# sohmandal/classpose

Measured on AMD Instinct MI355X. Metric: wsi_tiles_per_sec, higher is better.
Workload: dtype bf16; 1 GPU; configs[1]: synthetic 10000x10000 WSI (1936 tiles), tile 256 / overlap 32, conic 7 classes, ViT-L ClassTransformer depth 24 random-init, batch 32 sub-tiles = 8 WSI tiles/step, every step a distinct batch of the rank's shard (tiles sharded k % n_gpus, at most 256 distinct batches resident, longer runs wrap) streamed pinned host -> hipMemcpyAsync inside the timed region (the reader decodes ahead int; slide=10000, tile=256, overlap=32, batch_subtiles=32, distinct_batches=142, records_gathered=2048, decode_ahead_batches_at_t0=4, device_resident_batches_at_t0=1

## Files before the change

classpose_amd/csrc/cpx_gemm.hip:

```cpp
#include "cpx_internal.h"
#include <type_traits>

typedef __attribute__((ext_vector_type(8))) __bf16 bf16x8;
typedef __attribute__((ext_vector_type(8))) _Float16 f16x8;
typedef __attribute__((ext_vector_type(4))) float f32x4;

#define BM 128
#define BN 128
#define BK 64
#define GEMM_THREADS 256
#define TILE_BYTES (128 * 128)
#define STAGE_BYTES (2 * TILE_BYTES)

template <bool NT_POSSIBLE, bool WT_POSSIBLE = false>
__device__ __forceinline__ void st16(void *p, uint4 v, bool nt, bool wt = false) {
    if (WT_POSSIBLE && wt) {
        typedef unsigned u32x4_t __attribute__((ext_vector_type(4)));
        u32x4_t w = {v.x, v.y, v.z, v.w};
        if (NT_POSSIBLE && nt) asm volatile("global_store_dwordx4 %0, %1, off sc1 nt" ::"v"(p), "v"(w) : "memory");
        else asm volatile("global_store_dwordx4 %0, %1, off sc1" ::"v"(p), "v"(w) : "memory");
    } else if (NT_POSSIBLE && nt) {
        typedef unsigned u32x4_t __attribute__((ext_vector_type(4)));
        u32x4_t w = {v.x, v.y, v.z, v.w};
        __builtin_nontemporal_store(w, reinterpret_cast<u32x4_t *>(p));
// ... 228 lines not shown
                const size_t s_ = (size_t)(m >> 10), t_ = (size_t)(m & 1023);
#pragma unroll
                for (int r = 0; r < 4; ++r) {
                    const int c = n - 2048 + r;
                    vT[((s_ * 16 + (c >> 6)) * 64 + (c & 63)) * 1024 + t_] = to_half<F16>(v[r]);
                }
            } else {
                uint2 o;
                o.x = pack2<F16>(v[0], v[1]);
                o.y = pack2<F16>(v[2], v[3]);
                *reinterpret_cast<uint2 *>((unsigned short *)g.out + (size_t)m * g.ld_out + n) = o;
            }
        }
    }
}


typedef __attribute__((ext_vector_type(4))) unsigned u32x4;
#define G2_THREADS 512
#define G2_HALF 16384
#define G2_BUF 65536
#define G2_EPI_LD 528
#define G2_LN_OFF (256 * G2_EPI_LD)
#define G2_LDS_BYTES (G2_LN_OFF + 256 * 8)

template <int OFF>
__device__ __forceinline__ u32x4 lds_read128(unsigned addr) {
    u32x4 v;
    asm volatile("ds_read_b128 %0, %1 offset:%2" : "=v"(v) : "v"(addr), "n"(OFF));
    return v;
}
template <bool F16>
__device__ __forceinline__ f32x4 mfma16v(const u32x4 &a, const u32x4 &b, f32x4 c) {
    if constexpr (F16)
        return __builtin_amdgcn_mfma_f32_16x16x32_f16(__builtin_bit_cast(f16x8, a), __builtin_bit_cast(f16x8, b), c, 0, 0, 0);
    else
        return __builtin_amdgcn_mfma_f32_16x16x32_bf16(__builtin_bit_cast(bf16x8, a), __builtin_bit_cast(bf16x8, b), c, 0, 0, 0);
}
template <int HM>
__device__ __forceinline__ void g2_read_x(u32x4 (&fx)[4][2], unsigned b0, unsigned b1) {
    fx[0][0] = lds_read128<HM * G2_HALF + 0 * 2048>(b0); fx[0][1] = lds_read128<HM * G2_HALF + 0 * 2048>(b1);
    fx[1][0] = lds_read128<HM * G2_HALF + 1 * 2048>(b0); fx[1][1] = lds_read128<HM * G2_HALF + 1 * 2048>(b1);
    fx[2][0] = lds_read128<HM * G2_HALF + 2 * 2048>(b0); fx[2][1] = lds_read128<HM * G2_HALF + 2 * 2048>(b1);
    fx[3][0] = lds_read128<HM * G2_HALF + 3 * 2048>(b0); fx[3][1] = lds_read128<HM * G2_HALF + 3 * 2048>(b1);
}
template <int HN>
__device__ __forceinline__ void g2_read_w(u32x4 (&fw)[2][2], unsigned b0, unsigned b1) {
// ... 31 lines not shown
    int bid = blockIdx.x;
    {
        const int nxcd = 8, q = g.n_blocks / nxcd, r = g.n_blocks % nxcd, x = bid % nxcd;
        bid = (x < r ? x * (q + 1) : r * (q + 1) + (x - r) * q) + bid / nxcd;
    }
    int tile_m, tile_n;
    {
        const int tiles_m = g.n_blocks / g.tiles_n;
        if (g.l2_block && (tiles_m & 7) == 0 && (g.tiles_n & 3) == 0) {
            const int grp = bid >> 5, w_ = bid & 31, cgn = g.tiles_n >> 2, rgn = tiles_m >> 3;
            const int rg = g.l2_block == 2 ? grp % rgn : grp / cgn, cg = g.l2_block == 2 ? grp / rgn : grp - rg * cgn;
            tile_m = rg * 8 + (w_ >> 2);
            tile_n = cg * 4 + (w_ & 3);
        } else {
            tile_m = bid / g.tiles_n;
            tile_n = bid - tile_m * g.tiles_n;
        }
    }
    if (g.rev_m) tile_m = g.n_blocks / g.tiles_n - 1 - tile_m;
    const int m0 = tile_m * 256, n0 = tile_n * 256;
    const int K = g.K, nk = K / 64;

    const int srow = tid >> 3, kc = (tid & 7) ^ (srow & 7);
    const unsigned short *pX = g.A + (size_t)(m0 + srow) * K + kc * 8;
    const unsigned short *pW = g.W + (size_t)(n0 + srow) * K + kc * 8;
    const size_t k64 = (size_t)64 * K, k128 = (size_t)128 * K;
    char *sdst = smem + wave * 1024;
    auto stage = [&](int which, int t) {
        const unsigned short *p = (which < 2 ? pX : pW) + (which & 1) * k128 + (size_t)t * 64;
        char *d = sdst + (t & 1) * G2_BUF + which * G2_HALF;
        __builtin_amdgcn_global_load_lds((const __attribute__((address_space(1))) void *)p,
                                         (__attribute__((address_space(3))) void *)d, 16, 0, 0);
        __builtin_amdgcn_global_load_lds((const __attribute__((address_space(1))) void *)(p + k64),
                                         (__attribute__((address_space(3))) void *)(d + 8192), 16, 0, 0);
    };

    const unsigned lds0 = (unsigned)(size_t)(__attribute__((address_space(3))) char *)smem;
    unsigned xb[2][2], wb[2][2];
#pragma unroll
    for (int ks = 0; ks < 2; ++ks) {
        const unsigned sw = (unsigned)(((ks * 4 + fq) ^ (fr & 7)) << 4);
        xb[0][ks] = lds0 + (wm * 64 + fr) * 128 + sw;
        wb[0][ks] = lds0 + (wn * 32 + fr) * 128 + sw;
        xb[1][ks] = xb[0][ks] + G2_BUF;
        wb[1][ks] = wb[0][ks] + G2_BUF;
    }

    f32x4 acc[2][2][4][2];
#pragma unroll
    for (int a = 0; a < 2; ++a)
#pragma unroll
        for (int b = 0; b < 2; ++b)
#pragma unroll
            for (int c = 0; c < 4; ++c)
#pragma unroll
                for (int d = 0; d < 2; ++d) acc[a][b][c][d] = (f32x4){0.f, 0.f, 0.f, 0.f};
    u32x4 fx[4][2], fw[2][2];

    const bool ln_in = LN_IN && tid < 256;
    float4 st_a = make_float4(0.f, 0.f, 0.f, 0.f), st_b = st_a;
    if (ln_in) {
        st_a = *reinterpret_cast<const float4 *>(g.ln_stats + (size_t)(m0 + tid) * 8);
        st_b = *reinterpret_cast<const float4 *>(g.ln_stats + (size_t)(m0 + tid) * 8 + 4);
    }
    stage(0, 0); stage(2, 0); stage(3, 0); stage(1, 0);
    if (nk > 1) { stage(0, 1); stage(3, 1); }
    if (ln_in) {
        const float inv_k = 1.0f / K;
        const float sum = (st_a.x + st_a.z) + (st_b.x + st_b.z), sq = (st_a.y + st_a.w) + (st_b.y + st_b.w);
        const float mean = sum * inv_k;
        const float rstd = rsqrtf(fmaxf(sq * inv_k - mean * mean, 0.f) + 1e-6f);
        *reinterpret_cast<float2 *>(smem + G2_LN_OFF + tid * 8) = make_float2(rstd, -mean * rstd);
        asm volatile("s_waitcnt lgkmcnt(0)" ::: "memory");
    }
    if (nk > 1) asm volatile("s_waitcnt vmcnt(4)" ::: "memory");
    else asm volatile("s_waitcnt vmcnt(0)" ::: "memory");
    G2_BAR();
    if (wm == 1) G2_BAR();

#define G2_TILE(T, B)                                                                       \
    {                                                                                       \
        const int t_ = (T);                                                                 \
                                                                                    \
        g2_read_w<0>(fw, wb[B][0], wb[B][1]);                                               \
        g2_read_x<0>(fx, xb[B][0], xb[B][1]);                                               \
        if (t_ + 1 < nk) stage(1, t_ + 1);                                                  \
        G2_BAR(); G2_LGKM0();                                                               \
        g2_mma<F16>(acc[0][0], fx, fw);                                                     \
        __builtin_amdgcn_sched_barrier(0); G2_BAR();                                        \
                                                                                    \
        g2_read_w<1>(fw, wb[B][0], wb[B][1]);                                               \
        if (t_ + 1 < nk) stage(2, t_ + 1);                                                  \
        G2_BAR(); G2_LGKM0();                                                               \
        g2_mma<F16>(acc[0][1], fx, fw);                                                     \
        __builtin_amdgcn_sched_barrier(0); G2_BAR();                                        \
// ... 1 lines not shown
        g2_read_x<1>(fx, xb[B][0], xb[B][1]);                                               \
        if (t_ + 2 < nk) stage(0, t_ + 2);                                                  \
        G2_BAR(); G2_LGKM0();                                                               \
        g2_mma<F16>(acc[1][1], fx, fw);                                                     \
        __builtin_amdgcn_sched_barrier(0); G2_BAR();                                        \
                                                                                    \
        g2_read_w<0>(fw, wb[B][0], wb[B][1]);                                               \
        if (t_ + 2 < nk) { stage(3, t_ + 2); asm volatile("s_waitcnt vmcnt(4)" ::: "memory"); } \
        else if (t_ + 1 < nk) asm volatile("s_waitcnt vmcnt(0)" ::: "memory");              \
        G2_BAR(); G2_LGKM0();                                                               \
        g2_mma<F16>(acc[1][0], fx, fw);                                                     \
        __builtin_amdgcn_sched_barrier(0); G2_BAR();                                        \
    }

    for (int t = 0; t + 1 < nk; t += 2) {
        G2_TILE(t, 0)
        G2_TILE(t + 1, 1)
    }
    if (nk & 1) G2_TILE(nk - 1, 0)
#undef G2_TILE
    if (wm == 0) G2_BAR();
    __builtin_amdgcn_sched_barrier(0);

    const bool vt_tile = (EPI == CPX_EPI_QKV_BF16) && n0 >= 2048;
    const int c16 = tid & 31;
    float ln_mean[2][4], ln_rstd[2][4];
    if constexpr (LN_IN) {
#pragma unroll
        for (int hm = 0; hm < 2; ++hm)
#pragma unroll
            for (int mb = 0; mb < 4; ++mb) {
                const float2 p = *reinterpret_cast<const float2 *>(smem + G2_LN_OFF + (hm * 128 + wm * 64 + mb * 16 + fr) * 8);
                ln_rstd[hm][mb] = p.x; ln_mean[hm][mb] = p.y;
            }
    }
    uint4 rres[16];
    if constexpr (EPI == CPX_EPI_RESID_BF16) {
#pragma unroll
        for (int it = 0; it < 16; ++it)
            rres[it] = *reinterpret_cast<const uint4 *>((const unsigned short *)g.aux +
                                                        (size_t)(m0 + it * 16 + (tid >> 5)) * g.ld_out + n0 + c16 * 8);
    }
    float4 colb[2][2], colc[2][2];
#pragma unroll
    for (int hn = 0; hn < 2; ++hn)
#pragma unroll
        for (int nb = 0; nb < 2; ++nb) {
            const int nl = hn * 128 + wn * 32 + nb * 16 + fq * 4;
            colb[hn][nb] = g.bias ? *reinterpret_cast<const float4 *>(g.bias + n0 + nl) : make_float4(0.f, 0.f, 0.f, 0.f);
            if constexpr (LN_IN) colc[hn][nb] = *reinterpret_cast<const float4 *>(g.ln_colsum + n0 + nl);
        }
    auto convert_and_stage = [&](auto vt_tag) {
        constexpr bool VT = decltype(vt_tag)::value;
#pragma unroll
    for (int hm = 0; hm < 2; ++hm)
#pragma unroll
        for (int hn = 0; hn < 2; ++hn)
#pragma unroll
            for (int mb = 0; mb < 4; ++mb)
#pragma unroll
                for (int nb = 0; nb < 2; ++nb) {
                    const int ml = hm * 128 + wm * 64 + mb * 16 + fr;
                    const int nl = hn * 128 + wn * 32 + nb * 16 + fq * 4;
                    f32x4 v = acc[hm][hn][mb][nb];
                    const float4 b = colb[hn][nb];
                    if constexpr (LN_IN) {
                        const float4 cs = colc[hn][nb];
                        const float nm = ln_mean[hm][mb], rs = ln_rstd[hm][mb];
                        v[0] = fmaf(v[0], rs, fmaf(nm, cs.x, b.x)); v[1] = fmaf(v[1], rs, fmaf(nm, cs.y, b.y));
                        v[2] = fmaf(v[2], rs, fmaf(nm, cs.z, b.z)); v[3] = fmaf(v[3], rs, fmaf(nm, cs.w, b.w));
                    } else {
                        v[0] += b.x; v[1] += b.y; v[2] += b.z; v[3] += b.w;
                    }
                    if constexpr (EPI == CPX_EPI_GELU_BF16) {
#pragma unroll
                        for (int r = 0; r < 4; ++r) v[r] = gelu_erf(v[r]);
                    } else if constexpr (EPI == CPX_EPI_RELU_BF16) {
#pragma unroll
                        for (int r = 0; r < 4; ++r) v[r] = fmaxf(v[r], 0.f);
                    } else if constexpr (EPI == CPX_EPI_POS_BF16) {
                        const float4 pe = *reinterpret_cast<const float4 *>((const float *)g.aux + (size_t)((m0 + ml) & 1023) * g.N + n0 + nl);
                        v[0] += pe.x; v[1] += pe.y; v[2] += pe.z; v[3] += pe.w;
                    }
                    if constexpr (VT) {
                        const unsigned p01 = pack2<F16>(v[0], v[1]), p23 = pack2<F16>(v[2], v[3]);
                        *reinterpret_cast<unsigned short *>(smem + (nl + 0) * G2_EPI_LD + ml * 2) = (unsigned short)p01;
                        *reinterpret_cast<unsigned short *>(smem + (nl + 1) * G2_EPI_LD + ml * 2) = (unsigned short)(p01 >> 16);
                        *reinterpret_cast<unsigned short *>(smem + (nl + 2) * G2_EPI_LD + ml * 2) = (unsigned short)p23;
                        *reinterpret_cast<unsigned short *>(smem + (nl + 3) * G2_EPI_LD + ml * 2) = (unsigned short)(p23 >> 16);
                    } else {
                        uint2 o;
                        o.x = pack2<F16>(v[0], v[1]);
                        o.y = pack2<F16>(v[2], v[3]);
                        *reinterpret_cast<uint2 *>(smem + ml * G2_EPI_LD + nl * 2) = o;
                    }
                }
    };
    if (EPI == CPX_EPI_QKV_BF16 && vt_tile) convert_and_stage(std::true_type{});
    else convert_and_stage(std::false_type{});
    __syncthreads();
    if (vt_tile) {
        unsigned short *vT = (unsigned short *)g.aux;
        const size_t s_ = (size_t)(m0 >> 10), t0 = (size_t)(m0 & 1023);
#pragma unroll 4
        for (int it = 0; it < 16; ++it) {
            const int row = it * 16 + (tid >> 5);
            const int c = n0 - 2048 + row;
            uint4 v = *reinterpret_cast<const uint4 *>(smem + row * G2_EPI_LD + c16 * 16);
            *reinterpret_cast<uint4 *>(vT + ((s_ * 16 + (c >> 6)) * 64 + (c & 63)) * 1024 + t0 + c16 * 8) = v;
        }
    } else {
#pragma unroll
        for (int it = 0; it < 16; ++it) {
            const int ml = it * 16 + (tid >> 5);
            uint4 v = *reinterpret_cast<const uint4 *>(smem + ml * G2_EPI_LD + c16 * 16);
            const size_t go = (size_t)(m0 + ml) * g.ld_out + n0 + c16 * 8;
            if constexpr (EPI == CPX_EPI_RESID_BF16) {
                const uint4 rr = rres[it];
// ... 19 lines not shown
                if (c16 == 16)
                    *reinterpret_cast<float2 *>(g.stats_out + ((size_t)(m0 + ml) * LN_SLOTS + tile_n) * 2) = make_float2(sm, sq);
            }
        }
    }
}


#define G2P_STG_OFF G2_BUF
#define G2P_TAIL G2_LN_OFF
#define G2P_LDS_BYTES (G2_LN_OFF + 4096)
template <int EPI, bool F16, int FLAGS>
__global__ void __launch_bounds__(G2_THREADS, 2) k_gemm256p(GemmArgs g) {
    constexpr bool LN_IN = (FLAGS & G2F_LN) != 0 && EPI != CPX_EPI_RESID_BF16;
    constexpr bool STATS = (FLAGS & G2F_STATS) != 0 && EPI == CPX_EPI_RESID_BF16;
    extern __shared__ __attribute__((aligned(16))) char smem[];
    const int wave = __builtin_amdgcn_readfirstlane((int)threadIdx.x >> 6);
    const int wm = wave >> 2, wn = wave & 3;
    const int K = g.K, nk = K / 64, nblk = g.n_blocks, tiles_m = g.n_blocks / g.tiles_n;
    auto coords = [&](int v, int &m0_, int &n0_, int &tn_) {
        const int nxcd = 8, q = nblk / nxcd, r = nblk % nxcd, x = v % nxcd;
        int bid = (x < r ? x * (q + 1) : r * (q + 1) + (x - r) * q) + v / nxcd;
        int tile_m, tile_n;
        if (EPI == CPX_EPI_QKV_BF16 && g.l2_block == 3) {
            const int x = v & 7, slot = (v >> 3) & 31, i = v >> 8, rx = tiles_m >> 3, full = rx >> 4;
            int rg, cg;
            if (i < 6 * full) {
                const int rnd = i / 6, j = i - rnd * 6;
                rg = 2 * rnd + (j < 4 ? j >> 1 : j - 4); cg = j < 4 ? j & 1 : 2;
            } else {
                const int j = i - 6 * full;
                rg = 2 * full; cg = j < 2 ? j : 2;
            }
            tile_m = x * rx + rg * 8 + (slot >> 2);
            tile_n = cg * 4 + (slot & 3);
        } else if (g.l2_block && (tiles_m & 7) == 0 && (g.tiles_n & 3) == 0) {
            const int grp = bid >> 5, w_ = bid & 31, cgn = g.tiles_n >> 2, rgn = tiles_m >> 3;
            const int rg = g.l2_block == 2 ? grp % rgn : grp / cgn, cg = g.l2_block == 2 ? grp / rgn : grp - rg * cgn;
            tile_m = rg * 8 + (w_ >> 2);
            tile_n = cg * 4 + (w_ & 3);
        } else {
            tile_m = bid / g.tiles_n;
            tile_n = bid - tile_m * g.tiles_n;
        }
        if (g.rev_m) tile_m = tiles_m - 1 - tile_m;
        m0_ = tile_m * 256; n0_ = tile_n * 256; tn_ = tile_n;
    };
    char *sdst = smem + wave * 1024;
    const __amdgpu_buffer_rsrc_t rsrcX = __builtin_amdgcn_make_buffer_rsrc((void *)g.A, 0, 0x7FFFFFFF, 0x00020000);
    const __amdgpu_buffer_rsrc_t rsrcW = __builtin_amdgcn_make_buffer_rsrc((void *)g.W, 0, 0x7FFFFFFF, 0x00020000);
    const unsigned k64b = (unsigned)K * 128u, k128b = (unsigned)K * 256u;
    auto stage_at = [&](unsigned voff, unsigned sX, unsigned sW, int which, int t) {
        const unsigned so = (which < 2 ? sX : sW) + (which & 1) * k128b + (unsigned)t * 128u;
        char *d = sdst + (t & 1) * G2_BUF + which * G2_HALF;
        if (which < 2) {
            __builtin_amdgcn_raw_ptr_buffer_load_lds(rsrcX, (__attribute__((address_space(3))) void *)d, 16, voff, so, 0, 0);
            __builtin_amdgcn_raw_ptr_buffer_load_lds(rsrcX, (__attribute__((address_space(3))) void *)(d + 8192), 16, voff, so + k64b, 0, 0);
        } else {
            __builtin_amdgcn_raw_ptr_buffer_load_lds(rsrcW, (__attribute__((address_space(3))) void *)d, 16, voff, so, 0, 0);
            __builtin_amdgcn_raw_ptr_buffer_load_lds(rsrcW, (__attribute__((address_space(3))) void *)(d + 8192), 16, voff, so + k64b, 0, 0);
        }
    };
    const unsigned lds0 = (unsigned)(size_t)(__attribute__((address_space(3))) char *)smem;
    int v = blockIdx.x, m0, n0, tile_n;
    coords(v, m0, n0, tile_n);
    bool prefetched = false;
    for (;;) {
        const int vn = v + (int)gridDim.x;
        const bool has_next = vn < nblk;
        int m0n = 0, n0n = 0, tile_nn = 0;
        if (has_next) coords(vn, m0n, n0n, tile_nn);
        int tid = threadIdx.x;
        asm volatile("" : "+v"(tid));
        const int lane = tid & 63, fr = lane & 15, fq = lane >> 4, c16 = tid & 31;
        const int srow = tid >> 3, kc = (tid & 7) ^ (srow & 7);
        unsigned xb[2][2], wb[2][2];
#pragma unroll
        for (int ks = 0; ks < 2; ++ks) {
            const unsigned sw = (unsigned)(((ks * 4 + fq) ^ (fr & 7)) << 4);
            xb[0][ks] = lds0 + (wm * 64 + fr) * 128 + sw;
            wb[0][ks] = lds0 + (wn * 32 + fr) * 128 + sw;
            xb[1][ks] = xb[0][ks] + G2_BUF;
            wb[1][ks] = wb[0][ks] + G2_BUF;
        }
        const unsigned voff = ((unsigned)srow * (unsigned)K + (unsigned)kc * 8u) * 2u;
        const unsigned sX = (unsigned)m0 * (unsigned)K * 2u, sW = (unsigned)n0 * (unsigned)K * 2u;
        auto stage = [&](int which, int t) { stage_at(voff, sX, sW, which, t); };
        float4 st_a = make_float4(0.f, 0.f, 0.f, 0.f), st_b = st_a;
        float bias_v = 0.f, csum_v = 0.f;
        if (tid < 256) {
            if (LN_IN) {
                st_a = *reinterpret_cast<const float4 *>(g.ln_stats + (size_t)(m0 + tid) * 8);
                st_b = *reinterpret_cast<const float4 *>(g.ln_stats + (size_t)(m0 + tid) * 8 + 4);
            }
        } else {
            if (g.bias) bias_v = g.bias[n0 + tid - 256];
            if (LN_IN) csum_v = g.ln_colsum[n0 + tid - 256];
        }
        auto park_tile_vectors = [&]() {
            if (tid < 256) {
                if (LN_IN) {
                    const float inv_k = 1.0f / K;
                    const float sum = (st_a.x + st_a.z) + (st_b.x + st_b.z), sq = (st_a.y + st_a.w) + (st_b.y + st_b.w);
                    const float mean = sum * inv_k;
                    const float rstd = rsqrtf(fmaxf(sq * inv_k - mean * mean, 0.f) + 1e-6f);
                    *reinterpret_cast<float2 *>(smem + G2P_TAIL + tid * 8) = make_float2(rstd, -mean * rstd);
                }
            } else {
                *reinterpret_cast<float *>(smem + G2P_TAIL + 2048 + (tid - 256) * 4) = bias_v;
                *reinterpret_cast<float *>(smem + G2P_TAIL + 3072 + (tid - 256) * 4) = csum_v;
            }
        };
        constexpr bool BAL = (FLAGS & G2F_BAL) != 0;
        if (prefetched) {
            park_tile_vectors();
            if (nk > 1) { stage(0, 1); stage(3, 1); if constexpr (BAL) stage(2, 1); }
        } else {
            stage(0, 0); stage(2, 0); stage(3, 0); stage(1, 0);
            if (nk > 1) { stage(0, 1); stage(3, 1); if constexpr (BAL) stage(2, 1); }
            park_tile_vectors();
        }
        asm volatile("s_waitcnt lgkmcnt(0)" ::: "memory");
        if constexpr (BAL) asm volatile("s_waitcnt vmcnt(6)" ::: "memory");
        else if (nk > 1) asm volatile("s_waitcnt vmcnt(4)" ::: "memory");
        else asm volatile("s_waitcnt vmcnt(0)" ::: "memory");
        G2_BAR();
        f32x4 acc[2][2][4][2];
        u32x4 fx[4][2], fw[2][2], fw2[2][2];
        if constexpr (BAL) g2_read_w<0>(fw, wb[0][0], wb[0][1]);
        if (wm == 1) G2_BAR();
// ... 61 lines not shown
        if constexpr (BAL) {
            G2_TILE_BAL(0, 0, true, 0, fw, fw2)
            G2_TILE_BAL(1, 1, false, 2, fw2, fw)
            for (int t = 2; t + 2 < nk; t += 2) {
                G2_TILE_BAL(t, 0, false, 2, fw, fw2)
                G2_TILE_BAL(t + 1, 1, false, 2, fw2, fw)
            }
            G2_TILE_BAL(nk - 2, 0, false, 3, fw, fw2)
            G2_TILE_BAL(nk - 1, 1, false, 4, fw2, fw)
        } else {
        G2_TILE_PLAIN(0, 0, true, -1)
        G2_TILE_PLAIN(1, 1, false, -1)
        for (int t = 2; t < nk; t += 2) {
            G2_TILE_PLAIN(t, 0, false, -1)
            G2_TILE_PLAIN(t + 1, 1, false, -1)
        }
        }
#undef G2_TILE_BAL
#undef G2_VM
#undef G2_TILE_PLAIN
        if (wm == 0) G2_BAR();
        __builtin_amdgcn_sched_barrier(0);

        const bool vt_tile = (EPI == CPX_EPI_QKV_BF16) && n0 >= 2048;
        bool next_issued = false;
        const unsigned sXn = (unsigned)m0n * (unsigned)K * 2u, sWn = (unsigned)n0n * (unsigned)K * 2u;
        auto prefetch_next = [&]() {
            stage_at(voff, sXn, sWn, 0, 0); stage_at(voff, sXn, sWn, 2, 0); stage_at(voff, sXn, sWn, 3, 0); stage_at(voff, sXn, sWn, 1, 0);
            next_issued = true;
        };
        if (vt_tile) {
#pragma unroll
            for (int hm = 0; hm < 2; ++hm)
#pragma unroll
                for (int hn = 0; hn < 2; ++hn)
#pragma unroll
                    for (int mb = 0; mb < 4; ++mb)
#pragma unroll
                        for (int nb = 0; nb < 2; ++nb) {
                            const int ml = hm * 128 + wm * 64 + mb * 16 + fr;
                            const int nl = hn * 128 + wn * 32 + nb * 16 + fq * 4;
                            f32x4 vv = acc[hm][hn][mb][nb];
                            const float4 b = *reinterpret_cast<const float4 *>(smem + G2P_TAIL + 2048 + nl * 4);
                            if constexpr (LN_IN) {
                                const float4 cs = *reinterpret_cast<const float4 *>(smem + G2P_TAIL + 3072 + nl * 4);
                                const float2 pr = *reinterpret_cast<const float2 *>(smem + G2P_TAIL + ml * 8);
                                vv[0] = fmaf(vv[0], pr.x, fmaf(pr.y, cs.x, b.x)); vv[1] = fmaf(vv[1], pr.x, fmaf(pr.y, cs.y, b.y));
                                vv[2] = fmaf(vv[2], pr.x, fmaf(pr.y, cs.z, b.z)); vv[3] = fmaf(vv[3], pr.x, fmaf(pr.y, cs.w, b.w));
                            } else {
                                vv[0] += b.x; vv[1] += b.y; vv[2] += b.z; vv[3] += b.w;
                            }
                            const unsigned p01 = pack2<F16>(vv[0], vv[1]), p23 = pack2<F16>(vv[2], vv[3]);
                            *reinterpret_cast<unsigned short *>(smem + (nl + 0) * G2_EPI_LD + ml * 2) = (unsigned short)p01;
                            *reinterpret_cast<unsigned short *>(smem + (nl + 1) * G2_EPI_LD + ml * 2) = (unsigned short)(p01 >> 16);
                            *reinterpret_cast<unsigned short *>(smem + (nl + 2) * G2_EPI_LD + ml * 2) = (unsigned short)p23;
                            *reinterpret_cast<unsigned short *>(smem + (nl + 3) * G2_EPI_LD + ml * 2) = (unsigned short)(p23 >> 16);
                        }
            asm volatile("s_waitcnt lgkmcnt(0)" ::: "memory");
            G2_BAR();
            unsigned short *vT = (unsigned short *)g.aux;
            const size_t s_ = (size_t)(m0 >> 10), t0 = (size_t)(m0 & 1023);
#pragma unroll 4
            for (int it = 0; it < 16; ++it) {
                const int row = it * 16 + (tid >> 5);
                const int c = n0 - 2048 + row;
                uint4 vv = *reinterpret_cast<const uint4 *>(smem + row * G2_EPI_LD + c16 * 16);
                st16<EPI == CPX_EPI_QKV_BF16, EPI == CPX_EPI_QKV_BF16>(vT + ((s_ * 16 + (c >> 6)) * 64 + (c & 63)) * 1024 + t0 + c16 * 8, vv, (g.nt_out & 4) != 0, (g.nt_out & 16) != 0);
            }
            asm volatile("s_waitcnt lgkmcnt(0)" ::: "memory");
            G2_BAR();
        } else if constexpr (EPI != CPX_EPI_RESID_BF16 && (FLAGS & G2F_DIRECT) != 0) {
            if (has_next) prefetch_next();
            const __amdgpu_buffer_rsrc_t rsrcO = __builtin_amdgcn_make_buffer_rsrc((void *)g.out, 0, 0x7FFFFFFF, 0x00020000);
            const unsigned ldb = (unsigned)g.ld_out * 2u;
            const unsigned ovoff = (unsigned)(wm * 64 + fr) * ldb + (unsigned)(wn * 32 + ((fq & 1) << 4) + ((fq >> 1) << 3)) * 2u;
            const unsigned so0 = (unsigned)m0 * ldb + (unsigned)n0 * 2u;
#pragma unroll
            for (int hm = 0; hm < 2; ++hm) {
                float ln_rs[4], ln_nm[4];
                if constexpr (LN_IN) {
#pragma unroll
                    for (int mb = 0; mb < 4; ++mb) {
                        const float2 pr = *reinterpret_cast<const float2 *>(smem + G2P_TAIL + (hm * 128 + wm * 64 + mb * 16 + fr) * 8);
                        ln_rs[mb] = pr.x; ln_nm[mb] = pr.y;
                    }
                }
#pragma unroll
                for (int hn = 0; hn < 2; ++hn) {
                    float4 b[2], cs[2];
#pragma unroll
                    for (int nb = 0; nb < 2; ++nb) {
                        const int nl = hn * 128 + wn * 32 + nb * 16 + fq * 4;
                        b[nb] = *reinterpret_cast<const float4 *>(smem + G2P_TAIL + 2048 + nl * 4);
                        cs[nb] = make_float4(0.f, 0.f, 0.f, 0.f);
// ... 11 lines not shown
                                vv[2] = fmaf(vv[2], rs, fmaf(nm, cs[nb].z, b[nb].z)); vv[3] = fmaf(vv[3], rs, fmaf(nm, cs[nb].w, b[nb].w));
                            } else {
                                vv[0] += b[nb].x; vv[1] += b[nb].y; vv[2] += b[nb].z; vv[3] += b[nb].w;
                            }
                            if constexpr (EPI == CPX_EPI_GELU_BF16) {
#pragma unroll
                                for (int r = 0; r < 4; ++r) vv[r] = gelu_erf(vv[r]);
                            } else if constexpr (EPI == CPX_EPI_RELU_BF16) {
#pragma unroll
                                for (int r = 0; r < 4; ++r) vv[r] = fmaxf(vv[r], 0.f);
                            }
                            pk[nb][0] = pack2<F16>(vv[0], vv[1]);
                            pk[nb][1] = pack2<F16>(vv[2], vv[3]);
                        }
                        const auto r0 = __builtin_amdgcn_permlane16_swap(pk[0][0], pk[1][0], false, false);
                        const auto r1 = __builtin_amdgcn_permlane16_swap(pk[0][1], pk[1][1], false, false);
                        const u32x4 o = {r0[0], r1[0], r0[1], r1[1]};
                        __builtin_amdgcn_raw_buffer_store_b128(o, rsrcO, ovoff, so0 + (unsigned)(hm * 128 + mb * 16) * ldb + (unsigned)hn * 256u, 0);
                    }
                }
            }
            G2_BAR();
        } else {
            if constexpr (EPI != CPX_EPI_RESID_BF16) {
                if (has_next) prefetch_next();
            }
            char *stg = smem + G2P_STG_OFF;
#pragma unroll
            for (int hm = 0; hm < 2; ++hm) {
                uint4 rres[8];
                if constexpr (EPI == CPX_EPI_RESID_BF16) {
#pragma unroll
                    for (int it = 0; it < 8; ++it)
                        rres[it] = *reinterpret_cast<const uint4 *>((const unsigned short *)g.aux +
                                                                    (size_t)(m0 + hm * 128 + it * 16 + (tid >> 5)) * g.ld_out + n0 + c16 * 8);
                }
                float ln_rs[4], ln_nm[4];
                if constexpr (LN_IN) {
#pragma unroll
                    for (int mb = 0; mb < 4; ++mb) {
                        const float2 pr = *reinterpret_cast<const float2 *>(smem + G2P_TAIL + (hm * 128 + wm * 64 + mb * 16 + fr) * 8);
                        ln_rs[mb] = pr.x; ln_nm[mb] = pr.y;
                    }
                }
#pragma unroll
                for (int hn = 0; hn < 2; ++hn)
#pragma unroll
                    for (int nb = 0; nb < 2; ++nb) {
                        const int nl = hn * 128 + wn * 32 + nb * 16 + fq * 4;
                        const float4 b = *reinterpret_cast<const float4 *>(smem + G2P_TAIL + 2048 + nl * 4);
                        float4 cs = make_float4(0.f, 0.f, 0.f, 0.f);
                        if constexpr (LN_IN) cs = *reinterpret_cast<const float4 *>(smem + G2P_TAIL + 3072 + nl * 4);
#pragma unroll
                        for (int mb = 0; mb < 4; ++mb) {
                            const int mlh = wm * 64 + mb * 16 + fr;
                            f32x4 vv = acc[hm][hn][mb][nb];
                            if constexpr (LN_IN) {
                                const float nm = ln_nm[mb], rs = ln_rs[mb];
                                vv[0] = fmaf(vv[0], rs, fmaf(nm, cs.x, b.x)); vv[1] = fmaf(vv[1], rs, fmaf(nm, cs.y, b.y));
                                vv[2] = fmaf(vv[2], rs, fmaf(nm, cs.z, b.z)); vv[3] = fmaf(vv[3], rs, fmaf(nm, cs.w, b.w));
                            } else {
                                vv[0] += b.x; vv[1] += b.y; vv[2] += b.z; vv[3] += b.w;
                            }
                            if constexpr (EPI == CPX_EPI_GELU_BF16) {
#pragma unroll
                                for (int r = 0; r < 4; ++r) vv[r] = gelu_erf(vv[r]);
                            } else if constexpr (EPI == CPX_EPI_RELU_BF16) {
#pragma unroll
                                for (int r = 0; r < 4; ++r) vv[r] = fmaxf(vv[r], 0.f);
                            }
                            uint2 o;
                            o.x = pack2<F16>(vv[0], vv[1]);
                            o.y = pack2<F16>(vv[2], vv[3]);
                            *reinterpret_cast<uint2 *>(stg + mlh * G2_EPI_LD + nl * 2) = o;
                        }
                    }
                asm volatile("s_waitcnt lgkmcnt(0)" ::: "memory");
                G2_BAR();
#pragma unroll
                for (int it = 0; it < 8; ++it) {
                    const int mlh = it * 16 + (tid >> 5);
                    uint4 vv = *reinterpret_cast<const uint4 *>(stg + mlh * G2_EPI_LD + c16 * 16);
                    const int ml = hm * 128 + mlh;
                    const size_t go = (size_t)(m0 + ml) * g.ld_out + n0 + c16 * 8;
                    if constexpr (EPI == CPX_EPI_RESID_BF16) {
                        const uint4 rr = rres[it];
                        unsigned a[4] = {vv.x, vv.y, vv.z, vv.w}, b[4] = {rr.x, rr.y, rr.z, rr.w};
#pragma unroll
                        for (int i = 0; i < 4; ++i) {
                            float lo = from_half<F16>(a[i] & 0xFFFF) + from_half<F16>(b[i] & 0xFFFF);
                            float hi = from_half<F16>(a[i] >> 16) + from_half<F16>(b[i] >> 16);
                            a[i] = pack2<F16>(lo, hi);
                        }
                        vv = make_uint4(a[0], a[1], a[2], a[3]);
                    }
                    st16<EPI == CPX_EPI_QKV_BF16, EPI == CPX_EPI_RESID_BF16 || EPI == CPX_EPI_QKV_BF16>((unsigned short *)g.out + go, vv, (g.nt_out & (n0 < 1024 ? 1 : 2)) != 0,
                                                                                        (g.nt_out & (EPI == CPX_EPI_QKV_BF16 ? 16 : 8)) != 0);
                    if constexpr (STATS) {
                        unsigned a[4] = {vv.x, vv.y, vv.z, vv.w};
                        float sm = 0.f, sq = 0.f;
#pragma unroll
                        for (int i = 0; i < 4; ++i) {
                            const float lo = from_half<F16>(a[i] & 0xFFFF), hi = from_half<F16>(a[i] >> 16);
                            sm += lo + hi; sq += lo * lo + hi * hi;
                        }
                        sm = half_wave_sum(sm); sq = half_wave_sum(sq);
                        if (c16 == 16)
                            *reinterpret_cast<float2 *>(g.stats_out + ((size_t)(m0 + ml) * LN_SLOTS + tile_n) * 2) = make_float2(sm, sq);
                    }
                }
                asm volatile("s_waitcnt lgkmcnt(0)" ::: "memory");
                G2_BAR();
            }
        }
        if (!has_next) break;
        prefetched = next_issued;
        v = vn; m0 = m0n; n0 = n0n; tile_n = tile_nn;
    }
}

CPX_SWITCH(g_gemm_persist, 1);
CPX_SWITCH(g_gemm_variant, 1);
CPX_SWITCH(g_gemm_l2, 1);
CPX_SWITCH(g_gemm_persist_qkv, 1);
CPX_SWITCH(g_gemm_rev, 0);
CPX_SWITCH(g_gemm_big, 1);
CPX_SWITCH(g_gemm_bal, 1);
CPX_SWITCH(g_gemm_direct, 1);
CPX_SWITCH(g_gemm_nt, 15);
CPX_SWITCH(g_gemm_4w, 1);
#ifdef CPX_DEBUG
extern "C" void cpx_gemm_set_persistent(int on) { g_gemm_persist = on; }
extern "C" void cpx_gemm_set_variant(int glds) { g_gemm_variant = glds; }
extern "C" void cpx_gemm_set_persistent_qkv(int on) { g_gemm_persist_qkv = on; }
extern "C" void cpx_gemm_set_l2_block(int on) { g_gemm_l2 = on; }
extern "C" void cpx_gemm_set_reverse(int on) { g_gemm_rev = on; }
extern "C" void cpx_gemm_set_big(int on) { g_gemm_big = on; }
extern "C" void cpx_gemm_set_direct(int on) { g_gemm_direct = on; }
extern "C" void cpx_gemm_set_balanced(int on) { g_gemm_bal = on; }
extern "C" void cpx_gemm_set_4w(int on) { g_gemm_4w = on; }
extern "C" void cpx_gemm_set_nt(int on) { g_gemm_nt = on; }
#endif

template <int EPI, bool F16, int FLAGS>
static void launch_gemm256_flags(const GemmArgs &a, hipStream_t s) {
    const bool qkv_balanced = EPI == CPX_EPI_QKV_BF16 && g_gemm_persist_qkv && (a.n_blocks / a.tiles_n) % 64 == 0 && a.tiles_n == 12;
    const bool fits32 = (size_t)a.M * (size_t)a.K * 2 < ((size_t)1 << 31) && (size_t)a.N * (size_t)a.K * 2 < ((size_t)1 << 31);
    if (g_gemm_persist && fits32 && (EPI != CPX_EPI_QKV_BF16 || qkv_balanced)) {
        static CpxOncePerDevice once_p;
        static int n_cu = 0;
        once_p([] {
            (void)hipFuncSetAttribute((const void *)k_gemm256p<EPI, F16, FLAGS>, hipFuncAttributeMaxDynamicSharedMemorySize, G2P_LDS_BYTES);
            int dev = 0, cus = 256;
            (void)hipGetDevice(&dev);
            (void)hipDeviceGetAttribute(&cus, hipDeviceAttributeMultiprocessorCount, dev);
            n_cu = cus > 0 ? cus : 256;
        });
        if (EPI == CPX_EPI_QKV_BF16) {
            if (n_cu == 256) {
                GemmArgs b = a;
                b.l2_block = 3;
                hipLaunchKernelGGL((k_gemm256p<EPI, F16, FLAGS>), dim3(256), dim3(G2_THREADS), G2P_LDS_BYTES, s, b);
                return;
            }
        } else {
            const int grid = a.n_blocks < n_cu ? a.n_blocks : n_cu;
            hipLaunchKernelGGL((k_gemm256p<EPI, F16, FLAGS>), dim3(grid), dim3(G2_THREADS), G2P_LDS_BYTES, s, a);
            return;
        }
    }
    static CpxOncePerDevice once;
    once([] { (void)hipFuncSetAttribute((const void *)k_gemm256<EPI, F16, FLAGS>, hipFuncAttributeMaxDynamicSharedMemorySize, G2_LDS_BYTES); });
    hipLaunchKernelGGL((k_gemm256<EPI, F16, FLAGS>), dim3(a.n_blocks), dim3(G2_THREADS), G2_LDS_BYTES, s, a);
}

template <int EPI, bool F16>
static bool launch_gemm256(const GemmArgs &a0, hipStream_t s) {
    if constexpr (EPI == CPX_EPI_F32) return false;
    else {
        if (!g_gemm_big || a0.M % 256 || a0.N % 256 || a0.K < 128) return false;
        if ((a0.K / 64) % 2 && EPI != CPX_EPI_POS_BF16) return false;
        if ((a0.M / 256) * (a0.N / 256) < 256) return false;
        GemmArgs a = a0;
        a.tiles_n = a.N / 256; a.n_blocks = (a.M / 256) * (a.N / 256);
        constexpr bool PRODUCER = EPI == CPX_EPI_RESID_BF16 || EPI == CPX_EPI_POS_BF16;
        constexpr int F1 = PRODUCER ? G2F_STATS : G2F_LN;
        const bool f1 = PRODUCER ? a.stats_out != nullptr : a.ln_stats != nullptr;
        if constexpr (EPI == CPX_EPI_POS_BF16) {
            static CpxOncePerDevice once_pos;
            once_pos([] {
                (void)hipFuncSetAttribute((const void *)k_gemm256<EPI, F16, 0>, hipFuncAttributeMaxDynamicSharedMemorySize, G2_LDS_BYTES);
                (void)hipFuncSetAttribute((const void *)k_gemm256<EPI, F16, G2F_STATS>, hipFuncAttributeMaxDynamicSharedMemorySize, G2_LDS_BYTES);
// ... 183 lines not shown
```

Before: 377.0 tiles/s.

## Compute V tiles of QKV GEMM transposed by swapping operands, drop custom QKV schedule

For QKV GEMM tiles that produce V (n0 >= 2048), the kernel swaps the A and W operand pointers and buffer descriptors so the MFMA accumulators come out already transposed. The epilogue can then write V^T rows directly through the regular row-staged path, replacing the scattered 2-byte transposed LDS writes. Bias and LN column sums become per-row values for these tiles, and LN mean and rstd become per-column, so the LDS tail layout changes and grows. The QKV-specific persistent launch (fixed grid of 256, custom l2_block=3 tile order) is replaced by the generic persistent launch, trading that tuned tile order for simplicity.

```diff
diff --git a/classpose_amd/csrc/cpx_gemm.hip b/classpose_amd/csrc/cpx_gemm.hip
--- a/classpose_amd/csrc/cpx_gemm.hip
+++ b/classpose_amd/csrc/cpx_gemm.hip
@@ -274,7 +274,7 @@
 #define G2_BUF 65536
 #define G2_EPI_LD 528
 #define G2_LN_OFF (256 * G2_EPI_LD)
-#define G2_LDS_BYTES (G2_LN_OFF + 256 * 8)
+#define G2_LDS_BYTES (G2_LN_OFF + 4096)
 
 template <int OFF>
 __device__ __forceinline__ u32x4 lds_read128(unsigned addr) {
@@ -352,8 +352,9 @@
     const int K = g.K, nk = K / 64;
 
     const int srow = tid >> 3, kc = (tid & 7) ^ (srow & 7);
-    const unsigned short *pX = g.A + (size_t)(m0 + srow) * K + kc * 8;
-    const unsigned short *pW = g.W + (size_t)(n0 + srow) * K + kc * 8;
+    const bool vt_tile = (EPI == CPX_EPI_QKV_BF16) && n0 >= 2048;
+    const unsigned short *pX = (vt_tile ? g.W + (size_t)(n0 + srow) * K : g.A + (size_t)(m0 + srow) * K) + kc * 8;
+    const unsigned short *pW = (vt_tile ? g.A + (size_t)(m0 + srow) * K : g.W + (size_t)(n0 + srow) * K) + kc * 8;
     const size_t k64 = (size_t)64 * K, k128 = (size_t)128 * K;
     char *sdst = smem + wave * 1024;
     auto stage = [&](int which, int t) {
@@ -393,6 +394,11 @@
         st_a = *reinterpret_cast<const float4 *>(g.ln_stats + (size_t)(m0 + tid) * 8);
         st_b = *reinterpret_cast<const float4 *>(g.ln_stats + (size_t)(m0 + tid) * 8 + 4);
     }
+    float vbias = 0.f, vcsum = 0.f;
+    if (vt_tile && tid >= 256) {
+        if (g.bias) vbias = g.bias[n0 + tid - 256];
+        if constexpr (LN_IN) vcsum = g.ln_colsum[n0 + tid - 256];
+    }
     stage(0, 0); stage(2, 0); stage(3, 0); stage(1, 0);
     if (nk > 1) { stage(0, 1); stage(3, 1); }
     if (ln_in) {
@@ -400,7 +406,16 @@
         const float sum = (st_a.x + st_a.z) + (st_b.x + st_b.z), sq = (st_a.y + st_a.w) + (st_b.y + st_b.w);
         const float mean = sum * inv_k;
         const float rstd = rsqrtf(fmaxf(sq * inv_k - mean * mean, 0.f) + 1e-6f);
-        *reinterpret_cast<float2 *>(smem + G2_LN_OFF + tid * 8) = make_float2(rstd, -mean * rstd);
+        if (vt_tile) {
+            *reinterpret_cast<float *>(smem + G2_LN_OFF + 2048 + tid * 4) = rstd;
+            *reinterpret_cast<float *>(smem + G2_LN_OFF + 3072 + tid * 4) = -mean * rstd;
+        } else {
+            *reinterpret_cast<float2 *>(smem + G2_LN_OFF + tid * 8) = make_float2(rstd, -mean * rstd);
+        }
+        asm volatile("s_waitcnt lgkmcnt(0)" ::: "memory");
+    }
+    if (vt_tile && tid >= 256) {
+        *reinterpret_cast<float2 *>(smem + G2_LN_OFF + (tid - 256) * 8) = make_float2(vbias, vcsum);
         asm volatile("s_waitcnt lgkmcnt(0)" ::: "memory");
     }
     if (nk > 1) asm volatile("s_waitcnt vmcnt(4)" ::: "memory");
@@ -448,10 +463,9 @@
     if (wm == 0) G2_BAR();
     __builtin_amdgcn_sched_barrier(0);
 
-    const bool vt_tile = (EPI == CPX_EPI_QKV_BF16) && n0 >= 2048;
     const int c16 = tid & 31;
     float ln_mean[2][4], ln_rstd[2][4];
-    if constexpr (LN_IN) {
+    if (LN_IN || vt_tile) {
 #pragma unroll
         for (int hm = 0; hm < 2; ++hm)
 #pragma unroll
@@ -473,6 +487,13 @@
 #pragma unroll
         for (int nb = 0; nb < 2; ++nb) {
             const int nl = hn * 128 + wn * 32 + nb * 16 + fq * 4;
+            if (vt_tile) {
+                if constexpr (LN_IN) {
+                    colb[hn][nb] = *reinterpret_cast<const float4 *>(smem + G2_LN_OFF + 2048 + nl * 4);
+                    colc[hn][nb] = *reinterpret_cast<const float4 *>(smem + G2_LN_OFF + 3072 + nl * 4);
+                }
+                continue;
+            }
             colb[hn][nb] = g.bias ? *reinterpret_cast<const float4 *>(g.bias + n0 + nl) : make_float4(0.f, 0.f, 0.f, 0.f);
             if constexpr (LN_IN) colc[hn][nb] = *reinterpret_cast<const float4 *>(g.ln_colsum + n0 + nl);
         }
@@ -490,7 +511,15 @@
                     const int nl = hn * 128 + wn * 32 + nb * 16 + fq * 4;
                     f32x4 v = acc[hm][hn][mb][nb];
                     const float4 b = colb[hn][nb];
-                    if constexpr (LN_IN) {
+                    if constexpr (VT && LN_IN) {
+                        const float4 cs = colc[hn][nb];
+                        const float rc = ln_mean[hm][mb], rb = ln_rstd[hm][mb];
+                        v[0] = fmaf(v[0], b.x, fmaf(cs.x, rc, rb)); v[1] = fmaf(v[1], b.y, fmaf(cs.y, rc, rb));
+                        v[2] = fmaf(v[2], b.z, fmaf(cs.z, rc, rb)); v[3] = fmaf(v[3], b.w, fmaf(cs.w, rc, rb));
+                    } else if constexpr (VT) {
+                        const float rb = ln_rstd[hm][mb];
+                        v[0] += rb; v[1] += rb; v[2] += rb; v[3] += rb;
+                    } else if constexpr (LN_IN) {
                         const float4 cs = colc[hn][nb];
                         const float nm = ln_mean[hm][mb], rs = ln_rstd[hm][mb];
                         v[0] = fmaf(v[0], rs, fmaf(nm, cs.x, b.x)); v[1] = fmaf(v[1], rs, fmaf(nm, cs.y, b.y));
@@ -508,18 +537,10 @@
                         const float4 pe = *reinterpret_cast<const float4 *>((const float *)g.aux + (size_t)((m0 + ml) & 1023) * g.N + n0 + nl);
                         v[0] += pe.x; v[1] += pe.y; v[2] += pe.z; v[3] += pe.w;
                     }
-                    if constexpr (VT) {
-                        const unsigned p01 = pack2<F16>(v[0], v[1]), p23 = pack2<F16>(v[2], v[3]);
-                        *reinterpret_cast<unsigned short *>(smem + (nl + 0) * G2_EPI_LD + ml * 2) = (unsigned short)p01;
-                        *reinterpret_cast<unsigned short *>(smem + (nl + 1) * G2_EPI_LD + ml * 2) = (unsigned short)(p01 >> 16);
-                        *reinterpret_cast<unsigned short *>(smem + (nl + 2) * G2_EPI_LD + ml * 2) = (unsigned short)p23;
-                        *reinterpret_cast<unsigned short *>(smem + (nl + 3) * G2_EPI_LD + ml * 2) = (unsigned short)(p23 >> 16);
-                    } else {
-                        uint2 o;
-                        o.x = pack2<F16>(v[0], v[1]);
-                        o.y = pack2<F16>(v[2], v[3]);
-                        *reinterpret_cast<uint2 *>(smem + ml * G2_EPI_LD + nl * 2) = o;
-                    }
+                    uint2 o;
+                    o.x = pack2<F16>(v[0], v[1]);
+                    o.y = pack2<F16>(v[2], v[3]);
+                    *reinterpret_cast<uint2 *>(smem + ml * G2_EPI_LD + nl * 2) = o;
                 }
     };
     if (EPI == CPX_EPI_QKV_BF16 && vt_tile) convert_and_stage(std::true_type{});
@@ -585,19 +606,7 @@
         const int nxcd = 8, q = nblk / nxcd, r = nblk % nxcd, x = v % nxcd;
         int bid = (x < r ? x * (q + 1) : r * (q + 1) + (x - r) * q) + v / nxcd;
         int tile_m, tile_n;
-        if (EPI == CPX_EPI_QKV_BF16 && g.l2_block == 3) {
-            const int x = v & 7, slot = (v >> 3) & 31, i = v >> 8, rx = tiles_m >> 3, full = rx >> 4;
-            int rg, cg;
-            if (i < 6 * full) {
-                const int rnd = i / 6, j = i - rnd * 6;
-                rg = 2 * rnd + (j < 4 ? j >> 1 : j - 4); cg = j < 4 ? j & 1 : 2;
-            } else {
-                const int j = i - 6 * full;
-                rg = 2 * full; cg = j < 2 ? j : 2;
-            }
-            tile_m = x * rx + rg * 8 + (slot >> 2);
-            tile_n = cg * 4 + (slot & 3);
-        } else if (g.l2_block && (tiles_m & 7) == 0 && (g.tiles_n & 3) == 0) {
+        if (g.l2_block && (tiles_m & 7) == 0 && (g.tiles_n & 3) == 0) {
             const int grp = bid >> 5, w_ = bid & 31, cgn = g.tiles_n >> 2, rgn = tiles_m >> 3;
             const int rg = g.l2_block == 2 ? grp % rgn : grp / cgn, cg = g.l2_block == 2 ? grp / rgn : grp - rg * cgn;
             tile_m = rg * 8 + (w_ >> 2);
@@ -613,15 +622,17 @@
     const __amdgpu_buffer_rsrc_t rsrcX = __builtin_amdgcn_make_buffer_rsrc((void *)g.A, 0, 0x7FFFFFFF, 0x00020000);
     const __amdgpu_buffer_rsrc_t rsrcW = __builtin_amdgcn_make_buffer_rsrc((void *)g.W, 0, 0x7FFFFFFF, 0x00020000);
     const unsigned k64b = (unsigned)K * 128u, k128b = (unsigned)K * 256u;
-    auto stage_at = [&](unsigned voff, unsigned sX, unsigned sW, int which, int t) {
-        const unsigned so = (which < 2 ? sX : sW) + (which & 1) * k128b + (unsigned)t * 128u;
+    auto stage_at = [&](bool swap, unsigned voff, unsigned s01, unsigned s23, int which, int t) {
+        const unsigned so = (which < 2 ? s01 : s23) + (which & 1) * k128b + (unsigned)t * 128u;
         char *d = sdst + (t & 1) * G2_BUF + which * G2_HALF;
         if (which < 2) {
-            __builtin_amdgcn_raw_ptr_buffer_load_lds(rsrcX, (__attribute__((address_space(3))) void *)d, 16, voff, so, 0, 0);
-            __builtin_amdgcn_raw_ptr_buffer_load_lds(rsrcX, (__attribute__((address_space(3))) void *)(d + 8192), 16, voff, so + k64b, 0, 0);
+            const __amdgpu_buffer_rsrc_t r = (EPI == CPX_EPI_QKV_BF16 && swap) ? rsrcW : rsrcX;
+            __builtin_amdgcn_raw_ptr_buffer_load_lds(r, (__attribute__((address_space(3))) void *)d, 16, voff, so, 0, 0);
+            __builtin_amdgcn_raw_ptr_buffer_load_lds(r, (__attribute__((address_space(3))) void *)(d + 8192), 16, voff, so + k64b, 0, 0);
         } else {
-            __builtin_amdgcn_raw_ptr_buffer_load_lds(rsrcW, (__attribute__((address_space(3))) void *)d, 16, voff, so, 0, 0);
-            __builtin_amdgcn_raw_ptr_buffer_load_lds(rsrcW, (__attribute__((address_space(3))) void *)(d + 8192), 16, voff, so + k64b, 0, 0);
+            const __amdgpu_buffer_rsrc_t r = (EPI == CPX_EPI_QKV_BF16 && swap) ? rsrcX : rsrcW;
+            __builtin_amdgcn_raw_ptr_buffer_load_lds(r, (__attribute__((address_space(3))) void *)d, 16, voff, so, 0, 0);
+            __builtin_amdgcn_raw_ptr_buffer_load_lds(r, (__attribute__((address_space(3))) void *)(d + 8192), 16, voff, so + k64b, 0, 0);
         }
     };
     const unsigned lds0 = (unsigned)(size_t)(__attribute__((address_space(3))) char *)smem;
@@ -648,7 +659,8 @@
         }
         const unsigned voff = ((unsigned)srow * (unsigned)K + (unsigned)kc * 8u) * 2u;
         const unsigned sX = (unsigned)m0 * (unsigned)K * 2u, sW = (unsigned)n0 * (unsigned)K * 2u;
-        auto stage = [&](int which, int t) { stage_at(voff, sX, sW, which, t); };
+        const bool vt_tile = (EPI == CPX_EPI_QKV_BF16) && n0 >= 2048;
+        auto stage = [&](int which, int t) { stage_at(vt_tile, voff, vt_tile ? sW : sX, vt_tile ? sX : sW, which, t); };
         float4 st_a = make_float4(0.f, 0.f, 0.f, 0.f), st_b = st_a;
         float bias_v = 0.f, csum_v = 0.f;
         if (tid < 256) {
@@ -667,8 +679,15 @@
                     const float sum = (st_a.x + st_a.z) + (st_b.x + st_b.z), sq = (st_a.y + st_a.w) + (st_b.y + st_b.w);
                     const float mean = sum * inv_k;
                     const float rstd = rsqrtf(fmaxf(sq * inv_k - mean * mean, 0.f) + 1e-6f);
-                    *reinterpret_cast<float2 *>(smem + G2P_TAIL + tid * 8) = make_float2(rstd, -mean * rstd);
+                    if (vt_tile) {
+                        *reinterpret_cast<float *>(smem + G2P_TAIL + 2048 + tid * 4) = rstd;
+                        *reinterpret_cast<float *>(smem + G2P_TAIL + 3072 + tid * 4) = -mean * rstd;
+                    } else {
+                        *reinterpret_cast<float2 *>(smem + G2P_TAIL + tid * 8) = make_float2(rstd, -mean * rstd);
+                    }
                 }
+            } else if (vt_tile) {
+                *reinterpret_cast<float2 *>(smem + G2P_TAIL + (tid - 256) * 8) = make_float2(bias_v, csum_v);
             } else {
                 *reinterpret_cast<float *>(smem + G2P_TAIL + 2048 + (tid - 256) * 4) = bias_v;
                 *reinterpret_cast<float *>(smem + G2P_TAIL + 3072 + (tid - 256) * 4) = csum_v;
@@ -776,54 +795,15 @@
         if (wm == 0) G2_BAR();
         __builtin_amdgcn_sched_barrier(0);
 
-        const bool vt_tile = (EPI == CPX_EPI_QKV_BF16) && n0 >= 2048;
         bool next_issued = false;
+        const bool vt_next = (EPI == CPX_EPI_QKV_BF16) && n0n >= 2048;
         const unsigned sXn = (unsigned)m0n * (unsigned)K * 2u, sWn = (unsigned)n0n * (unsigned)K * 2u;
+        const unsigned s01n = vt_next ? sWn : sXn, s23n = vt_next ? sXn : sWn;
         auto prefetch_next = [&]() {
-            stage_at(voff, sXn, sWn, 0, 0); stage_at(voff, sXn, sWn, 2, 0); stage_at(voff, sXn, sWn, 3, 0); stage_at(voff, sXn, sWn, 1, 0);
+            stage_at(vt_next, voff, s01n, s23n, 0, 0); stage_at(vt_next, voff, s01n, s23n, 2, 0); stage_at(vt_next, voff, s01n, s23n, 3, 0); stage_at(vt_next, voff, s01n, s23n, 1, 0);
             next_issued = true;
         };
-        if (vt_tile) {
-#pragma unroll
-            for (int hm = 0; hm < 2; ++hm)
-#pragma unroll
-                for (int hn = 0; hn < 2; ++hn)
-#pragma unroll
-                    for (int mb = 0; mb < 4; ++mb)
-#pragma unroll
-                        for (int nb = 0; nb < 2; ++nb) {
-                            const int ml = hm * 128 + wm * 64 + mb * 16 + fr;
-                            const int nl = hn * 128 + wn * 32 + nb * 16 + fq * 4;
-                            f32x4 vv = acc[hm][hn][mb][nb];
-                            const float4 b = *reinterpret_cast<const float4 *>(smem + G2P_TAIL + 2048 + nl * 4);
-                            if constexpr (LN_IN) {
-                                const float4 cs = *reinterpret_cast<const float4 *>(smem + G2P_TAIL + 3072 + nl * 4);
-                                const float2 pr = *reinterpret_cast<const float2 *>(smem + G2P_TAIL + ml * 8);
-                                vv[0] = fmaf(vv[0], pr.x, fmaf(pr.y, cs.x, b.x)); vv[1] = fmaf(vv[1], pr.x, fmaf(pr.y, cs.y, b.y));
-                                vv[2] = fmaf(vv[2], pr.x, fmaf(pr.y, cs.z, b.z)); vv[3] = fmaf(vv[3], pr.x, fmaf(pr.y, cs.w, b.w));
-                            } else {
-                                vv[0] += b.x; vv[1] += b.y; vv[2] += b.z; vv[3] += b.w;
-                            }
-                            const unsigned p01 = pack2<F16>(vv[0], vv[1]), p23 = pack2<F16>(vv[2], vv[3]);
-                            *reinterpret_cast<unsigned short *>(smem + (nl + 0) * G2_EPI_LD + ml * 2) = (unsigned short)p01;
-                            *reinterpret_cast<unsigned short *>(smem + (nl + 1) * G2_EPI_LD + ml * 2) = (unsigned short)(p01 >> 16);
-                            *reinterpret_cast<unsigned short *>(smem + (nl + 2) * G2_EPI_LD + ml * 2) = (unsigned short)p23;
-                            *reinterpret_cast<unsigned short *>(smem + (nl + 3) * G2_EPI_LD + ml * 2) = (unsigned short)(p23 >> 16);
-                        }
-            asm volatile("s_waitcnt lgkmcnt(0)" ::: "memory");
-            G2_BAR();
-            unsigned short *vT = (unsigned short *)g.aux;
-            const size_t s_ = (size_t)(m0 >> 10), t0 = (size_t)(m0 & 1023);
-#pragma unroll 4
-            for (int it = 0; it < 16; ++it) {
-                const int row = it * 16 + (tid >> 5);
-                const int c = n0 - 2048 + row;
-                uint4 vv = *reinterpret_cast<const uint4 *>(smem + row * G2_EPI_LD + c16 * 16);
-                st16<EPI == CPX_EPI_QKV_BF16, EPI == CPX_EPI_QKV_BF16>(vT + ((s_ * 16 + (c >> 6)) * 64 + (c & 63)) * 1024 + t0 + c16 * 8, vv, (g.nt_out & 4) != 0, (g.nt_out & 16) != 0);
-            }
-            asm volatile("s_waitcnt lgkmcnt(0)" ::: "memory");
-            G2_BAR();
-        } else if constexpr (EPI != CPX_EPI_RESID_BF16 && (FLAGS & G2F_DIRECT) != 0) {
+        if constexpr (EPI != CPX_EPI_RESID_BF16 && (FLAGS & G2F_DIRECT) != 0) {
             if (has_next) prefetch_next();
             const __amdgpu_buffer_rsrc_t rsrcO = __builtin_amdgcn_make_buffer_rsrc((void *)g.out, 0, 0x7FFFFFFF, 0x00020000);
             const unsigned ldb = (unsigned)g.ld_out * 2u;
@@ -881,6 +861,8 @@
             }
             G2_BAR();
         } else {
+            auto staged_rows = [&](auto vt_tag) {
+            constexpr bool VT = decltype(vt_tag)::value;
             if constexpr (EPI != CPX_EPI_RESID_BF16) {
                 if (has_next) prefetch_next();
             }
@@ -895,7 +877,7 @@
                                                                     (size_t)(m0 + hm * 128 + it * 16 + (tid >> 5)) * g.ld_out + n0 + c16 * 8);
                 }
                 float ln_rs[4], ln_nm[4];
-                if constexpr (LN_IN) {
+                if constexpr (LN_IN || VT) {
 #pragma unroll
                     for (int mb = 0; mb < 4; ++mb) {
                         const float2 pr = *reinterpret_cast<const float2 *>(smem + G2P_TAIL + (hm * 128 + wm * 64 + mb * 16 + fr) * 8);
@@ -914,7 +896,14 @@
                         for (int mb = 0; mb < 4; ++mb) {
                             const int mlh = wm * 64 + mb * 16 + fr;
                             f32x4 vv = acc[hm][hn][mb][nb];
-                            if constexpr (LN_IN) {
+                            if constexpr (VT && LN_IN) {
+                                const float rb = ln_rs[mb], rc = ln_nm[mb];
+                                vv[0] = fmaf(vv[0], b.x, fmaf(cs.x, rc, rb)); vv[1] = fmaf(vv[1], b.y, fmaf(cs.y, rc, rb));
+                                vv[2] = fmaf(vv[2], b.z, fmaf(cs.z, rc, rb)); vv[3] = fmaf(vv[3], b.w, fmaf(cs.w, rc, rb));
+                            } else if constexpr (VT) {
+                                const float rb = ln_rs[mb];
+                                vv[0] += rb; vv[1] += rb; vv[2] += rb; vv[3] += rb;
+                            } else if constexpr (LN_IN) {
                                 const float nm = ln_nm[mb], rs = ln_rs[mb];
                                 vv[0] = fmaf(vv[0], rs, fmaf(nm, cs.x, b.x)); vv[1] = fmaf(vv[1], rs, fmaf(nm, cs.y, b.y));
                                 vv[2] = fmaf(vv[2], rs, fmaf(nm, cs.z, b.z)); vv[3] = fmaf(vv[3], rs, fmaf(nm, cs.w, b.w));
@@ -953,6 +942,10 @@
                         }
                         vv = make_uint4(a[0], a[1], a[2], a[3]);
                     }
+                    if constexpr (VT)
+                        st16<true, true>((unsigned short *)g.aux + ((size_t)(m0 >> 10) * 1024 + (size_t)(n0 - 2048 + ml)) * 1024 + (m0 & 1023) + c16 * 8, vv,
+                                         (g.nt_out & 4) != 0, (g.nt_out & 16) != 0);
+                    else
                     st16<EPI == CPX_EPI_QKV_BF16, EPI == CPX_EPI_RESID_BF16 || EPI == CPX_EPI_QKV_BF16>((unsigned short *)g.out + go, vv, (g.nt_out & (n0 < 1024 ? 1 : 2)) != 0,
                                                                                         (g.nt_out & (EPI == CPX_EPI_QKV_BF16 ? 16 : 8)) != 0);
                     if constexpr (STATS) {
@@ -970,6 +963,13 @@
                 }
                 asm volatile("s_waitcnt lgkmcnt(0)" ::: "memory");
                 G2_BAR();
+            }
+            };
+            if constexpr (EPI == CPX_EPI_QKV_BF16) {
+                if (vt_tile) staged_rows(std::true_type{});
+                else staged_rows(std::false_type{});
+            } else {
+                staged_rows(std::false_type{});
             }
         }
         if (!has_next) break;
@@ -1003,9 +1003,8 @@
 
 template <int EPI, bool F16, int FLAGS>
 static void launch_gemm256_flags(const GemmArgs &a, hipStream_t s) {
-    const bool qkv_balanced = EPI == CPX_EPI_QKV_BF16 && g_gemm_persist_qkv && (a.n_blocks / a.tiles_n) % 64 == 0 && a.tiles_n == 12;
     const bool fits32 = (size_t)a.M * (size_t)a.K * 2 < ((size_t)1 << 31) && (size_t)a.N * (size_t)a.K * 2 < ((size_t)1 << 31);
-    if (g_gemm_persist && fits32 && (EPI != CPX_EPI_QKV_BF16 || qkv_balanced)) {
+    if (g_gemm_persist && fits32 && (EPI != CPX_EPI_QKV_BF16 || g_gemm_persist_qkv)) {
         static CpxOncePerDevice once_p;
         static int n_cu = 0;
         once_p([] {
@@ -1015,18 +1014,9 @@
             (void)hipDeviceGetAttribute(&cus, hipDeviceAttributeMultiprocessorCount, dev);
             n_cu = cus > 0 ? cus : 256;
         });
-        if (EPI == CPX_EPI_QKV_BF16) {
-            if (n_cu == 256) {
-                GemmArgs b = a;
-                b.l2_block = 3;
-                hipLaunchKernelGGL((k_gemm256p<EPI, F16, FLAGS>), dim3(256), dim3(G2_THREADS), G2P_LDS_BYTES, s, b);
-                return;
-            }
-        } else {
-            const int grid = a.n_blocks < n_cu ? a.n_blocks : n_cu;
-            hipLaunchKernelGGL((k_gemm256p<EPI, F16, FLAGS>), dim3(grid), dim3(G2_THREADS), G2P_LDS_BYTES, s, a);
-            return;
-        }
+        const int grid = a.n_blocks < n_cu ? a.n_blocks : n_cu;
+        hipLaunchKernelGGL((k_gemm256p<EPI, F16, FLAGS>), dim3(grid), dim3(G2_THREADS), G2P_LDS_BYTES, s, a);
+        return;
     }
     static CpxOncePerDevice once;
     once([] { (void)hipFuncSetAttribute((const void *)k_gemm256<EPI, F16, FLAGS>, hipFuncAttributeMaxDynamicSharedMemorySize, G2_LDS_BYTES); });
```

New measurement: 378.9 tiles/s, median of 6. About the same (+0.5%).
